# open-mmlab/Amphion

Hardware: AMD Instinct MI355X
Metric: audio samples/sec (HiFi-GAN V1 22.05 kHz generator, mel->wav) (higher is better)
Workload: dtype f32 (split-f16 MFMA: 3 x v_mfma_f32_32x32x16_f16 per term, f32 accumulate)

## Files before the change

amphion_amd/csrc/conv_host.hip:

```cpp
#include <string.h>

#include <memory>
#include <type_traits>
#include <vector>

#include "amp_host.h"

namespace amp {

template <int... K> struct Taps { static constexpr int list[] = {K...}; };
using ConvTaps = Taps<1, 2, 3, 5, 7, 11>;
using BlkTaps = Taps<2, 3, 7, 11>;
using SmallTaps = Taps<1, 3, 5, 7, 11>;
using PairTaps = Taps<3, 5, 7, 11>;
using RbTaps = Taps<3, 5, 7, 11>;
using AmpbTaps = Taps<3, 5, 7, 11>;

template <int... K, typename R, typename F>
static R with_taps(Taps<K...>, int k, R dflt, F&& f) {
    R r = dflt;
    (void)((k == K && (r = f(std::integral_constant<int, K>{}), true)) || ...);
    return r;
}

static hipError_t launch_conv(const ConvPlan& p, const ConvArgs& a, hipStream_t s) {
    return with_taps(ConvTaps{}, p.KT, hipErrorInvalidValue, [&](auto K) { return launch_conv<K>(p, a, s); });
}
static hipError_t launch_conv_f16x3(const ConvPlan& p, const ConvArgs& a, hipStream_t s) {
    return with_taps(ConvTaps{}, p.KT, hipErrorInvalidValue, [&](auto K) { return launch_conv_f16x3<K>(p, a, s); });
}
static int conv_blk_nt(int k, int cm, int halo) { return with_taps(BlkTaps{}, k, 0, [&](auto K) { return conv_blk_nt<K>(cm, halo); }); }
static hipError_t launch_conv_blk(int k, int cm, int wn, const ConvArgs& a, hipStream_t s) {
    return with_taps(BlkTaps{}, k, hipErrorInvalidValue, [&](auto K) { return launch_conv_blk<K>(cm, wn, a, s); });
}
static hipError_t launch_conv_small(int k, int ni, int epi, const ConvArgs& a, hipStream_t s) {
    return with_taps(SmallTaps{}, k, hipErrorInvalidValue, [&](auto K) { return launch_conv_small<K>(ni, epi, a, s); });
}
static int pair_tile(int k, int C, int dil) { return with_taps(PairTaps{}, k, 0, [&](auto K) { return pair_tile<K>(C, dil); }); }
static hipError_t launch_pair(int k, const PairArgs& a, hipStream_t s) {
    return with_taps(PairTaps{}, k, hipErrorInvalidValue, [&](auto K) { return launch_pair<K>(a, s); });
}
static int strip_step(int k, int C, int dil, int wide, int* wg) {
    return with_taps(PairTaps{}, k, 0, [&](auto K) { return strip_step<K>(C, dil, wide, wg); });
}
static hipError_t launch_strip(int k, const PairArgs& a, hipStream_t s) {
    return with_taps(PairTaps{}, k, hipErrorInvalidValue, [&](auto K) { return launch_strip<K>(a, s); });
}
static int rb_tile(int k, int C, int max_dil, int wide) { return with_taps(RbTaps{}, k, 0, [&](auto K) { return rb_tile<K>(C, max_dil, wide); }); }
static hipError_t launch_rb(int k, const RbArgs& a, int wide, hipStream_t s) {
    return with_taps(RbTaps{}, k, hipErrorInvalidValue, [&](auto K) { return launch_rb<K>(a, wide, s); });
}
static int ampb_tile(int k, int C, int max_dil, int wide) {
    return with_taps(AmpbTaps{}, k, 0, [&](auto K) { return ampb_tile<K>(C, max_dil, wide); });
}
static hipError_t launch_ampb(int k, const AmpbArgs& a, int wide, hipStream_t s) {
    return with_taps(AmpbTaps{}, k, hipErrorInvalidValue, [&](auto K) { return launch_ampb<K>(a, wide, s); });
}

static int round_up_taps(int ntaps) {
    for (int kt : ConvTaps::list)
        if (kt >= ntaps) return kt;
    return -1;
}

bool choose_plan(int KT, int M, int halo_total, int , ConvPlan* plan) {
    bool ok = false;
    for (int kt : ConvTaps::list) ok |= (kt == KT);
    if (!ok || halo_total > 128) return false;
    plan->KT = KT;
    plan->HALO = halo_total <= 64 ? 64 : 128;
    if (M > 64) { plan->WM = 4; plan->WN = 1; plan->NI = 8; }
    else if (M > 32) { plan->WM = 2; plan->WN = 2; plan->NI = 8; }
    else { plan->WM = 1; plan->WN = 4; plan->NI = 4; }
    return true;
}

struct StripChoice { bool use; int wide; int steps; };
static StripChoice strip_choice(int C, int k) {
    const int mode = cfg().pair_strips;
    if (mode == 0) return {false, 0, 0};
    if (C == 128 && (k == 7 || k == 11)) return {true, 3, 1};
    return {false, 0, 0};
}

static void strip_plan(int B, int T, int n1, int hb, int wg_per_cu, int* strip_len, int* spi_out) {
    const int slots = wg_per_cu * 256;
    long best = -1; int best_spi = 1;
    const int max_spi = (T + n1 - 1) / n1;
    for (int spi = 1; spi <= max_spi; ++spi) {
        const int L = (T + spi - 1) / spi;
        if ((long)(spi - 1) * L >= T) continue;
        const long steps = (L + hb + n1 - 1) / n1;
        const long rounds = ((long)B * spi + slots - 1) / slots;
        const long cost = rounds * (4 * steps + 1);
        if (best < 0 || cost < best) { best = cost; best_spi = spi; }
    }
    *spi_out = best_spi;
    *strip_len = (T + best_spi - 1) / best_spi;
}

constexpr double kFitPrologueSteps = 0.2;
static void strip_geometry(int B, int T, int n1, int hb, int wg_per_cu, int steps, bool ragged, int* strip_len, int* spi, int* fit) {
    *fit = 0;
    strip_plan(B, T, n1, hb, wg_per_cu, strip_len, spi);
    if (steps > 0 && steps * n1 - hb < T) { *strip_len = steps * n1 - hb; *spi = (T + *strip_len - 1) / *strip_len; }
    bool four = false;
    if (steps == 1 && !ragged && 4 * n1 - hb < T) {
        const int len4 = 4 * n1 - hb, spi4 = (T + len4 - 1) / len4;
        if ((long long)B * spi4 >= 1024) { *strip_len = len4; *spi = spi4; four = true; }
    }
    const int mode = cfg().strip_fit;
    if (mode == 0) return;
    if (mode == 1) {
        const int st = (*strip_len + hb + n1 - 1) / n1;
        *strip_len = st * n1; *spi = (T + *strip_len - 1) / *strip_len; *fit = 1;
        return;
    }
    if (!four) return;
    const long long slots = (long long)wg_per_cu * 256;
    auto rounds = [&](int nspi) { return ((long long)B * nspi + slots - 1) / slots; };
    auto cost = [&](int nspi, double steps_per_strip) { return (double)rounds(nspi) * (4.0 * steps_per_strip + 1.0); };
    double best = cost(*spi, 4.0);
    const long long shifted_rounds = rounds(*spi) * 4;
    for (int S : {4, 8}) {
        const int len = S * n1, nspi = (T + len - 1) / len;
        if (len > T || (long long)B * nspi < 512) continue;
        if (rounds(nspi) * S >= shifted_rounds) continue;
        const double c = cost(nspi, S + kFitPrologueSteps);
        if (c < best) { best = c; *strip_len = len; *spi = nspi; *fit = 1; }
    }
}

bool pair_strip_plan(int B, int T, int k, bool ragged, int* form, int* strip_len, int* spi, int* steps) {
    int wg = 2;
    const StripChoice sc = strip_choice(128, k);
    const int n1 = sc.use ? strip_step(k, 128, 1, sc.wide, &wg) : 0;
    if (n1 <= 0) return false;
    strip_geometry(B, T, n1, k - 1, wg, sc.steps, ragged, strip_len, spi, form);
    *steps = (*strip_len + (*form ? 0 : k - 1) + n1 - 1) / n1;
    return true;
}

constexpr long long kSmallGridWorkgroups = 384;

static bool small_conv_enabled() { return cfg().small_conv != 0; }

static int conv_blk_mode() { return cfg().conv_blk; }
static int narrow_blk_mode() { return cfg().narrow_blk; }
constexpr size_t kConvRgFastMaxWeightBytes = 3u << 20;
static bool conv_rg_fast() { return cfg().conv_rg_fast != 0; }
static thread_local unsigned g_launch_parity = 0;
int next_rev(const int* lens) {
    if (!cfg().pingpong || lens) return 0;
    return (int)(g_launch_parity++ & 1u);
}
constexpr long long kConvBlkMinWorkgroups = 512;

int conv_build(amp_conv* c, const float* w, const float* bias) {
    if (c->cin <= 0 || c->cout <= 0 || c->k <= 0 || c->stride <= 0 || c->dilation <= 0) {
        set_error("amp_conv: bad dimensions cin=%d cout=%d k=%d stride=%d dilation=%d", c->cin, c->cout, c->k, c->stride,
                  c->dilation);
        return AMP_ERR_INVALID;
    }
    if (!c->transposed) {
        if (c->stride != 1) { set_error("amp_conv: strided Conv1d is not on the vocoder path"); return AMP_ERR_UNSUPPORTED; }
        c->up = 1; c->up_pad = 0;
        c->M = c->cout;
        c->ntaps = c->k;
        c->off0 = -c->padding;
        c->dstep = c->dilation;
    } else if (c->stride == 1) {
        if (c->dilation != 1) { set_error("amp_conv: dilated ConvTranspose1d unsupported (dilation=%d)", c->dilation); return AMP_ERR_UNSUPPORTED; }
        c->up = 1; c->up_pad = 0;
        c->M = c->cout;
        c->ntaps = c->k;
        c->off0 = -(c->k - 1 - c->padding);
        c->dstep = 1;
    } else {
        if (c->dilation != 1) { set_error("amp_conv: dilated ConvTranspose1d unsupported (dilation=%d)", c->dilation); return AMP_ERR_UNSUPPORTED; }
        c->up = c->stride; c->up_pad = c->padding;
        c->M = c->cout * c->stride;
        c->ntaps = (c->k + c->stride - 1) / c->stride;
        c->off0 = 0;
        c->dstep = -1;
    }
    c->KT = round_up_taps(c->ntaps);
    if (c->KT < 0) { set_error("amp_conv: k=%d at stride=%d is %d taps, unsupported (max 11)", c->k, c->stride, c->ntaps); return AMP_ERR_UNSUPPORTED; }
    const int omin = c->dstep >= 0 ? c->off0 : c->off0 + (c->KT - 1) * c->dstep;
    const int omax = c->dstep >= 0 ? c->off0 + (c->KT - 1) * c->dstep : c->off0;
    c->halo_left = omin < 0 ? -omin : 0;
    c->halo_right = omax > 0 ? omax : 0;
    if (!choose_plan(c->KT, c->M, c->halo_left + c->halo_right, 0, &c->plan)) {
        set_error("amp_conv: receptive field (k=%d, dilation=%d, padding=%d: %d columns) exceeds the 128-column staged halo", c->k, c->dilation,
                  c->padding, c->halo_left + c->halo_right);
        return AMP_ERR_UNSUPPORTED;
    }
    c->precision = default_precision();
    if (c->precision == PREC_F16X3) c->plan.NI = 4;
    const int Mg = c->plan.Mgroup();
    const int Mpad = ((c->M + Mg - 1) / Mg) * Mg;
    c->Mpad = Mpad;
    const int nmb = Mpad / 32;
    const int cin = c->cin, cout = c->cout, k = c->k, up = c->up;
    auto wview = [&](int m, int i, int g) -> float {
        if (m >= c->M || i >= cin || g >= c->ntaps) return 0.f;
        if (!c->transposed) return w[((size_t)m * cin + i) * k + g];
        if (up == 1) return w[((size_t)i * cout + m) * k + (k - 1 - g)];
        const int o = m / up, r = m - o * up;
        const int j = r + g * up;
        return j < k ? w[((size_t)i * cout + o) * k + j] : 0.f;
    };
    if (c->precision == PREC_F32) {
        c->nchunks = (c->cin + KC - 1) / KC;
        const size_t n = ((size_t)nmb * c->nchunks + 1) * c->KT * 64 * 4;
        std::vector<float> wp(n, 0.f);
        for (int mb = 0; mb < nmb; ++mb)
            for (int ch = 0; ch < c->nchunks; ++ch)
                for (int g = 0; g < c->KT; ++g)
                    for (int lane = 0; lane < 64; ++lane)
                        for (int p = 0; p < 4; ++p)
                            wp[((((size_t)mb * c->nchunks + ch) * c->KT + g) * 64 + lane) * 4 + p] =
                                wview(mb * 32 + (lane & 31), ch * KC + 2 * p + (lane >> 5), g);
        AMP_RC(device_upload(wp.data(), n * sizeof(float), &c->wp_dev));
    } else {
        c->nchunks = (c->cin + KC16 - 1) / KC16;
        float wmax = 0.f;
        const size_t nw = (size_t)cin * cout * k;
        for (size_t i = 0; i < nw; ++i) wmax = fmaxf(wmax, fabsf(w[i]));
        if (!(wmax < 1e30f)) { set_error("amp_conv: non-finite weight"); return AMP_ERR_INVALID; }
        c->wscale = pow2_weight_scale(wmax);
        const std::vector<_Float16> wp = pack_a_f16x3(nmb, c->nchunks, c->KT, (size_t)2 * c->KT * 2, c->wscale, wview);
        AMP_RC(device_upload(wp.data(), wp.size() * sizeof(_Float16), &c->wp_dev));
    }
    if (bias) AMP_RC(device_upload(bias, (size_t)cout * sizeof(float), (void**)&c->bias_dev));
    return AMP_OK;
}

static size_t conv_weight_bytes(const amp_conv* c) { return (size_t)c->Mpad * c->nchunks * KC16 * c->KT * 4; }

static int conv_out_len(const amp_conv* c, int T) {
    if (!c->transposed) return T + 2 * c->padding - c->dilation * (c->k - 1);
    return (T - 1) * c->stride - 2 * c->padding + c->k + c->out_pad;
}

static bool small_conv_static_ok(const amp_conv* c) {
    return c->precision == PREC_F16X3 && !c->transposed && !c->pad_reflect && c->plan.WM == 4 &&
           (c->KT == 1 || c->KT == 3 || c->KT == 5 || c->KT == 7 || c->KT == 11) && c->KT == c->ntaps &&
           c->nchunks <= kSmallConvMaxChunks && c->halo_left + c->halo_right <= 64;
}
static bool small_conv_covers(const amp_conv* c) { return small_conv_enabled() && small_conv_static_ok(c); }
static int small_conv_ni(const amp_conv* c) { return (c->halo_left + c->halo_right <= 32) ? 1 : 2; }

int conv_run(const amp_conv* c, const float* x, int B, int T, float slope_in, const float* res, float slope_out,
             float* y, int mode, float div, hipStream_t stream, long long xbs, const int* lens, int len_mul,
             ConvArgs* plan_small, int* plan_ni) {
    if (B <= 0 || T <= 0) { set_error("amp_conv_forward: B=%d T=%d", B, T); return AMP_ERR_INVALID; }
    const int Tout = conv_out_len(c, T);
    if (Tout <= 0) { set_error("amp_conv_forward: input too short (T=%d gives T_out=%d)", T, Tout); return AMP_ERR_INVALID; }
    ConvArgs a{};
    a.x = x; a.wp = c->wp_dev; a.bias = c->bias_dev; a.res = res; a.y = y;
    a.B = B; a.Cin = c->cin; a.Tin = T; a.xbs = xbs > 0 ? xbs : (long long)c->cin * T; a.nchunks = c->nchunks; a.M = c->M;
    a.Tq = c->up > 1 ? T + c->ntaps - 1 : Tout;
    ConvPlan plan = c->plan;
    if (c->precision == PREC_F16X3) {
        const long long wgs = (long long)B * ((a.Tq + plan.NT() - 1) / plan.NT()) * ((c->M + plan.Mgroup() - 1) / plan.Mgroup());
        if (wgs < kSmallGridWorkgroups) plan.NI = 2;
    }
    const int NT = plan.NT();
    a.tiles_per_item = (a.Tq + NT - 1) / NT;
    a.off0 = c->off0; a.dstep = c->dstep; a.halo_left = c->halo_left;
    a.wd = NT + c->halo_left + c->halo_right;
    a.Cout = c->cout; a.Tout = Tout; a.up = c->up; a.up_pad = c->up_pad;
    a.slope_in = slope_in; a.slope_out = slope_out; a.mode = mode; a.div = div;
    a.lens = lens; a.len_mul = len_mul;
    a.pad_reflect = c->pad_reflect; a.tanh_out = c->tanh_out;
    a.range_flag = c->precision == PREC_F16X3 ? range_flag_for_current_device() : nullptr;
    a.rev = c->precision == PREC_F16X3 ? next_rev(lens) : 0;
    if (c->pad_reflect && (c->halo_left >= T || c->halo_right >= T)) {
        set_error("amp_conv_forward: reflection padding %d needs more than %d input samples", c->halo_left > c->halo_right ? c->halo_left : c->halo_right, T);
        return AMP_ERR_INVALID;
    }
    if (c->gated_H) { set_error("amp_conv_forward: a gated conv (amp_conv_create_gated) only runs inside amp_wn_forward"); return AMP_ERR_STATE; }
    if (c->precision == PREC_F16X3 && slope_in > 1.f) {
        set_error("amp_conv_forward: leaky_relu slope %g > 1 on the input is outside the f16x3 kernels (use AMP_PRECISION_F32)", (double)slope_in);
        return AMP_ERR_UNSUPPORTED;
    }
    tl_conv_transposed = c->transposed;
    if (c->precision == PREC_F32) {
        if (plan_small) return AMP_ERR_UNSUPPORTED;
        a.acc_scale = a.inv_scale = 1.f;
        AMP_HIP(launch_conv(plan, a, stream));
    } else {
        a.acc_scale = 16.f * c->wscale;
        a.inv_scale = 1.f / a.acc_scale;
        const long long wgs_half = (long long)B * ((a.Tq + 63) / 64) * ((c->M + plan.Mgroup() - 1) / plan.Mgroup());
        int blk_cm = 0, blk_nt = 0, blk_wn = 1;
        const bool blk_kt = c->KT == 2 || c->KT == 3 || (conv_blk_mode() == 3 && (c->KT == 7 || c->KT == 11));
        if (c->M % 256 == 0) blk_wn = 1;
        else if (c->M % 128 == 0 && c->KT != 2 && (narrow_blk_mode() >= 2 || (narrow_blk_mode() == 1 && c->KT >= 7))) blk_wn = 2;
        else blk_wn = 0;
        if (conv_blk_mode() > 0 && plan.NI == 4 && blk_wn > 0 && blk_kt && !c->tanh_out && !c->pad_reflect) {
            int cm = (conv_blk_mode() >= 2 && c->KT == 2 && c->nchunks % 2 == 0) ? 2 : 1;
            const int halo = c->halo_left + c->halo_right;
            const int nt = blk_wn * conv_blk_nt(c->KT, cm, halo);
            if (nt > 0 && (long long)B * ((a.Tq + nt - 1) / nt) * (c->M / (256 / blk_wn)) >= kConvBlkMinWorkgroups) { blk_cm = cm; blk_nt = nt; }
        }
        if (plan_small && !(blk_cm == 0 && plan.NI == 2 && small_conv_covers(c) && (c->KT <= 5 || wgs_half <= 128))) return AMP_ERR_UNSUPPORTED;
        if (blk_cm > 0) {
            const int rows = 256 / blk_wn;
            a.tiles_per_item = (a.Tq + blk_nt - 1) / blk_nt;
            a.wd = blk_nt + c->halo_left + c->halo_right;
            a.row_groups = (conv_rg_fast() && c->M / rows > 1 && conv_weight_bytes(c) <= kConvRgFastMaxWeightBytes) ? c->M / rows : 0;
            AMP_HIP(launch_conv_blk(c->KT, blk_cm, blk_wn, a, stream));
        } else if (plan.NI == 2 && small_conv_covers(c) && (c->KT <= 5 || wgs_half <= 128)) {
            const int ni = small_conv_ni(c);
            a.Mpad = c->Mpad;
            a.tiles_per_item = (a.Tq + 32 * ni - 1) / (32 * ni);
            a.wd = 32 * ni + c->halo_left + c->halo_right;
            if (plan_small) { *plan_small = a; *plan_ni = ni; return AMP_OK; }
            AMP_HIP(launch_conv_small(c->KT, ni, 0, a, stream));
        } else {
            const int nrg = (c->M + plan.Mgroup() - 1) / plan.Mgroup();
            a.row_groups = (conv_rg_fast() && nrg > 1 && conv_weight_bytes(c) <= kConvRgFastMaxWeightBytes) ? nrg : 0;
            AMP_HIP(launch_conv_f16x3(plan, a, stream));
        }
    }
    return AMP_OK;
}

bool pair_supported(const amp_conv* c1, const amp_conv* c2) {
    if (c1->precision != PREC_F16X3 || c2->precision != PREC_F16X3) return false;
    if (c1->pad_reflect || c2->pad_reflect || c1->tanh_out || c2->tanh_out) return false;
    if (c1->transposed || c2->transposed || c1->cin != c1->cout || c2->cin != c2->cout || c1->cin != c2->cin) return false;
    if (c1->k != c2->k || c2->dilation != 1 || c1->k != c1->KT) return false;
    if (c1->padding != (c1->k - 1) / 2 * c1->dilation || c2->padding != (c2->k - 1) / 2) return false;
    if (!c1->bias_dev || !c2->bias_dev) return false;
    const StripChoice sc = strip_choice(c1->cin, c1->k);
    if (sc.use && strip_step(c1->k, c1->cin, c1->dilation, sc.wide, nullptr) > 0) return true;
    return pair_tile(c1->k, c1->cin, c1->dilation) > 0;
}

int pair_run(const amp_conv* c1, const amp_conv* c2, const float* x, int B, int T, float slope, float* y,
                    int mode, float div, hipStream_t stream, const int* lens, int len_mul) {
    if (x == y) { set_error("pair_run: x and y must not alias"); return AMP_ERR_INVALID; }
    if (slope > 1.f) { set_error("pair_run: leaky_relu slope %g > 1 is outside the fused pair kernels", (double)slope); return AMP_ERR_UNSUPPORTED; }
    PairArgs a{};
    a.x = x; a.y = y;
    a.wp1 = c1->wp_dev; a.bias1 = c1->bias_dev; a.wp2 = c2->wp_dev; a.bias2 = c2->bias_dev;
    a.B = B; a.C = c1->cin; a.T = T;
    a.dil = c1->dilation;
    a.slope = slope;
    a.sc1 = 16.f * c1->wscale; a.isc1 = 1.f / a.sc1;
    a.sc2 = 16.f * c2->wscale; a.isc2 = 1.f / a.sc2;
    a.mode = mode; a.div = div;
    a.lens = lens; a.len_mul = len_mul;
    a.range_flag = range_flag_for_current_device();
    a.rev = next_rev(lens);
    int wg = 2;
    const StripChoice sc = strip_choice(c1->cin, c1->k);
    const int n1 = sc.use ? strip_step(c1->k, c1->cin, c1->dilation, sc.wide, &wg) : 0;
    if (n1 > 0) {
        a.wide = sc.wide;
        strip_geometry(B, T, n1, c1->k - 1, wg, sc.steps, lens != nullptr, &a.strip_len, &a.strips_per_item, &a.fit);
        if (cfg().pair_strips == -1 && sc.wide >= 2 && (long long)B * a.strips_per_item < 512 && pair_tile(c1->k, c1->cin, c1->dilation) > 0) {
            const int NT = pair_tile(c1->k, c1->cin, c1->dilation);
            a.tiles_per_item = (T + NT - 1) / NT;
            AMP_HIP(launch_pair(c1->k, a, stream));
            return AMP_OK;
        }
        AMP_HIP(launch_strip(c1->k, a, stream));
        return AMP_OK;
    }
    const int NT = pair_tile(c1->k, c1->cin, c1->dilation);
    a.tiles_per_item = (T + NT - 1) / NT;
    AMP_HIP(launch_pair(c1->k, a, stream));
    return AMP_OK;
}

bool pair_tile_args(const amp_conv* c1, const amp_conv* c2, const float* x, int B, int T, float slope, float* y, int mode,
                           float div, const int* lens, int len_mul, PairArgs* out) {
    if (x == y || slope > 1.f || !pair_supported(c1, c2)) return false;
    PairArgs a{};
    a.x = x; a.y = y;
    a.wp1 = c1->wp_dev; a.bias1 = c1->bias_dev; a.wp2 = c2->wp_dev; a.bias2 = c2->bias_dev;
    a.B = B; a.C = c1->cin; a.T = T;
    a.dil = c1->dilation;
    a.slope = slope;
    a.sc1 = 16.f * c1->wscale; a.isc1 = 1.f / a.sc1;
    a.sc2 = 16.f * c2->wscale; a.isc2 = 1.f / a.sc2;
    a.mode = mode; a.div = div;
    a.lens = lens; a.len_mul = len_mul;
    a.range_flag = range_flag_for_current_device();
    a.rev = 0;
    int wg = 2;
    const StripChoice sc = strip_choice(c1->cin, c1->k);
    const int n1 = sc.use ? strip_step(c1->k, c1->cin, c1->dilation, sc.wide, &wg) : 0;
    if (n1 > 0) {
        int strip_len = 0, strips_per_item = 0, fit = 0;
        strip_geometry(B, T, n1, c1->k - 1, wg, sc.steps, lens != nullptr, &strip_len, &strips_per_item, &fit);
        if (!(cfg().pair_strips == -1 && sc.wide >= 2 && (long long)B * strips_per_item < 512)) return false;
    }
    const int NT = pair_tile(c1->k, c1->cin, c1->dilation);
    if (NT <= 0) return false;
    a.tiles_per_item = (T + NT - 1) / NT;
    *out = a;
    return true;
}

static int rb_fusion_mode() { return cfg().rb_fusion; }
static int rb_form(int C, int k) {
    const int m = rb_fusion_mode();
    if (m == 0) return -1;
    if (m == 3) return (C == 32 || (C == 64 && k <= 5)) ? 0 : 1;
    if (m == 2) return 1;
    if (C == 32) return k >= 11 ? 1 : 0;
    if (C == 64) return k <= 5 ? 0 : 1;
    if (C == 128) return 1;
    return -1;
}
constexpr long long kRbMinWorkgroups = 256;

bool rb_supported(const amp_conv* const* c1, const amp_conv* const* c2, int np, int B, int T) {
    if (np < 1 || np > AMP_RB_MAX_PAIRS) return false;
    int max_dil = 1, rh = 0;
    for (int p = 0; p < np; ++p) {
        if (!c1[p] || !c2[p] || !pair_supported(c1[p], c2[p])) return false;
        if (c1[p]->cin != c1[0]->cin || c1[p]->k != c1[0]->k) return false;
        max_dil = c1[p]->dilation > max_dil ? c1[p]->dilation : max_dil;
        rh += (c1[p]->k - 1) / 2 * (c1[p]->dilation + 1);
    }
    const int form = rb_form(c1[0]->cin, c1[0]->k);
    if (form < 0) return false;
    const int W = rb_tile(c1[0]->k, c1[0]->cin, max_dil, form);
    if (W <= 0 || W - 2 * rh < W / 2) return false;
    const int NT = W - 2 * rh;
    if (rb_fusion_mode() == 1 && (long long)B * ((T + NT - 1) / NT) < kRbMinWorkgroups) return false;
    return true;
}

int rb_split(const amp_conv* const* c1, int np, int B, int T) {
    if (np != 3 || rb_fusion_mode() != 1) return 0;
    int max_dil = 1, rh = 0;
    for (int p = 0; p < np; ++p) {
        max_dil = c1[p]->dilation > max_dil ? c1[p]->dilation : max_dil;
        rh += (c1[p]->k - 1) / 2 * (c1[p]->dilation + 1);
    }
    const int W = rb_tile(c1[0]->k, c1[0]->cin, max_dil, rb_form(c1[0]->cin, c1[0]->k));
    const int NT = W - 2 * rh;
    if (W <= 0 || 5 * NT >= 4 * W) return 0;
    if ((long long)B * ((T + NT - 1) / NT) < 1024) return 0;
    return 2;
}

int rb_run(const amp_conv* const* c1, const amp_conv* const* c2, int np, const float* x, int B, int T, float slope, float* y, int mode,
           float div, hipStream_t stream, const int* lens, int len_mul, int first, int count) {
    if (x == y) { set_error("rb_run: x and y must not alias"); return AMP_ERR_INVALID; }
    if (slope > 1.f) { set_error("rb_run: leaky_relu slope %g > 1 is outside the fused kernels", (double)slope); return AMP_ERR_UNSUPPORTED; }
    RbArgs a{};
    a.x = x; a.y = y;
    a.np = count < 0 ? np - first : count;
    c1 += first;
    c2 += first;
    int max_dil = 1;
    for (int p = 0; p < a.np; ++p) {
        a.wp1[p] = c1[p]->wp_dev; a.bias1[p] = c1[p]->bias_dev; a.wp2[p] = c2[p]->wp_dev; a.bias2[p] = c2[p]->bias_dev;
        a.sc1[p] = 16.f * c1[p]->wscale; a.isc1[p] = 1.f / a.sc1[p];
        a.sc2[p] = 16.f * c2[p]->wscale; a.isc2[p] = 1.f / a.sc2[p];
        a.dil[p] = c1[p]->dilation;
        a.rh += (c1[p]->k - 1) / 2 * (c1[p]->dilation + 1);
        max_dil = c1[p]->dilation > max_dil ? c1[p]->dilation : max_dil;
    }
    for (int p = a.np; p < AMP_RB_MAX_PAIRS; ++p) {
        a.wp1[p] = a.wp1[0]; a.bias1[p] = a.bias1[0]; a.wp2[p] = a.wp2[0]; a.bias2[p] = a.bias2[0]; a.dil[p] = 1;
    }
    a.B = B; a.C = c1[0]->cin; a.T = T;
    const int form = rb_form(a.C, c1[0]->k);
    const int W = rb_tile(c1[0]->k, a.C, max_dil, form);
    const int NT = W - 2 * a.rh;
    a.tiles_per_item = (T + NT - 1) / NT;
    a.slope = slope; a.mode = mode; a.div = div;
    a.lens = lens; a.len_mul = len_mul;
    a.range_flag = range_flag_for_current_device();
    a.rev = next_rev(lens);
    AMP_HIP(launch_rb(c1[0]->k, a, form, stream));
    return AMP_OK;
}

static int ampb_fusion_mode() { return cfg().ampb_fusion; }
static int ampb_form(int C, int k) {
    const int m = ampb_fusion_mode();
    if (m == 0) return -1;
    if (m == 3) return C == 32 ? 0 : 1;
    if (m == 2) return 1;
    if (C == 32) return k >= 11 ? 1 : 0;
    if (C == 64) return k <= 3 ? 1 : -1;
    return -1;
}
constexpr long long kAmpbMinWorkgroups = 256;

static int ampb_halo(const amp_conv* const* c1, int np) {
    int rh = 0;
    for (int p = 0; p < np; ++p) rh += 10 + (c1[p]->k - 1) / 2 * (c1[p]->dilation + 1);
    return (rh + 3) & ~3;
}

bool ampb_supported(const amp_conv* const* c1, const amp_conv* const* c2, int np, const ActParams* acts, size_t nacts, int B, int T) {
    if (np < 1 || 2 * np > AMP_AMPB_MAX_STEPS || nacts != (size_t)(2 * np)) return false;
    for (size_t i = 0; i < nacts; ++i)
        if (!acts[i].fu2_dev) return false;
    if ((T & 3) != 0) return false;
    int max_dil = 1;
    for (int p = 0; p < np; ++p) {
        const amp_conv *a = c1[p], *b = c2[p];
        if (!a || !b || a->precision != PREC_F16X3 || b->precision != PREC_F16X3) return false;
        if (a->pad_reflect || b->pad_reflect || a->tanh_out || b->tanh_out || a->transposed || b->transposed) return false;
        if (a->cin != a->cout || b->cin != b->cout || a->cin != b->cin || a->cin != c1[0]->cin) return false;
        if (a->k != c1[0]->k || b->k != a->k || b->dilation != 1 || a->k != a->KT) return false;
        if (a->padding != (a->k - 1) / 2 * a->dilation || b->padding != (b->k - 1) / 2) return false;
        if (!a->bias_dev || !b->bias_dev) return false;
        max_dil = a->dilation > max_dil ? a->dilation : max_dil;
    }
    const int form = ampb_form(c1[0]->cin, c1[0]->k);
    if (form < 0) return false;
    const int W = ampb_tile(c1[0]->k, c1[0]->cin, max_dil, form);
    const int rh = ampb_halo(c1, np);
    if (W <= 0 || W - 2 * rh < W / 2) return false;
    const int NT = W - 2 * rh;
    if (ampb_fusion_mode() == 1 && (long long)B * ((T + NT - 1) / NT) < kAmpbMinWorkgroups) return false;
    return true;
}

int ampb_run(const amp_conv* const* c1, const amp_conv* const* c2, int np, const ActParams* acts, const float* x, int B, int T,
                    float* y, int mode, float div, hipStream_t stream, const int* lens, int len_mul) {
    if (x == y) { set_error("ampb_run: x and y must not alias"); return AMP_ERR_INVALID; }
    AmpbArgs a{};
    a.x = x; a.y = y;
    a.ns = 2 * np;
    int max_dil = 1;
    for (int s = 0; s < AMP_AMPB_MAX_STEPS; ++s) {
        const int sv = s < a.ns ? s : 0;
        const amp_conv* c = (sv & 1) ? c2[sv >> 1] : c1[sv >> 1];
        a.wp[s] = c->wp_dev; a.bias[s] = c->bias_dev;
        a.sc[s] = 16.f * c->wscale; a.isc[s] = 1.f / a.sc[s];
        a.dil[s] = c->dilation;
        a.act_a[s] = acts[sv].a_dev; a.act_invb[s] = acts[sv].invb_dev; a.act_fu[s] = acts[sv].fu2_dev; a.act_fd[s] = acts[sv].fd_dev;
        max_dil = c->dilation > max_dil ? c->dilation : max_dil;
    }
    a.rh = ampb_halo(c1, np);
    a.B = B; a.C = c1[0]->cin; a.T = T;
    const int form = ampb_form(a.C, c1[0]->k);
    const int W = ampb_tile(c1[0]->k, a.C, max_dil, form);
    const int NT = W - 2 * a.rh;
    a.tiles_per_item = (T + NT - 1) / NT;
    a.mode = mode; a.div = div;
    a.lens = lens; a.len_mul = len_mul;
    a.range_flag = range_flag_for_current_device();
    a.rev = next_rev(lens);
    AMP_HIP(launch_ampb(c1[0]->k, a, form, stream));
    return AMP_OK;
}

int act_params_upload(const float* alpha_dev, const float* beta_dev, int C, int logscale, const float* filt_up_host,
                             const float* filt_down_host, float** out) {
    std::vector<float> al(C), be(C), a(C), ib(C);
    AMP_HIP(hipMemcpy(al.data(), alpha_dev, C * sizeof(float), hipMemcpyDeviceToHost));
    if (beta_dev) AMP_HIP(hipMemcpy(be.data(), beta_dev, C * sizeof(float), hipMemcpyDeviceToHost));
    for (int i = 0; i < C; ++i) {
        float av = al[i], bv = beta_dev ? be[i] : al[i];
        if (logscale) { av = expf(av); bv = expf(bv); }
        a[i] = av;
        ib[i] = 1.0f / (bv + 0.000000001f);
    }
    float* scratch = nullptr;
    AMP_HIP(hipMalloc((void**)&scratch, (2 * (size_t)C + 36) * sizeof(float)));
    float fu2[12];
    for (int i = 0; i < 12; ++i) fu2[i] = 2.f * filt_up_host[i];
    hipError_t e = hipMemcpy(scratch, a.data(), C * sizeof(float), hipMemcpyHostToDevice);
    if (e == hipSuccess) e = hipMemcpy(scratch + C, ib.data(), C * sizeof(float), hipMemcpyHostToDevice);
    if (e == hipSuccess) e = hipMemcpy(scratch + 2 * C, filt_up_host, 12 * sizeof(float), hipMemcpyHostToDevice);
    if (e == hipSuccess) e = hipMemcpy(scratch + 2 * C + 12, filt_down_host, 12 * sizeof(float), hipMemcpyHostToDevice);
    if (e == hipSuccess) e = hipMemcpy(scratch + 2 * C + 24, fu2, 12 * sizeof(float), hipMemcpyHostToDevice);
    if (e != hipSuccess) { (void)hipFree(scratch); set_error("act_params_upload: %s", hipGetErrorString(e)); return AMP_ERR_HIP; }
    *out = scratch;
    return AMP_OK;
}

}

using namespace amp;

extern "C" {

int amp_conv_create(int transposed, int cin, int cout, int k, int stride, int dilation, int padding,
                    const float* weight_host, const float* bias_host, amp_conv** out) {
    if (!weight_host || !out) { set_error("amp_conv_create: null argument"); return AMP_ERR_INVALID; }
    if (amp_device_count() <= 0) { set_error("amp_conv_create: no HIP device visible (the HIP path has no CPU fallback)"); return AMP_ERR_HIP; }
    auto c = std::make_unique<amp_conv>();
    c->transposed = transposed; c->cin = cin; c->cout = cout; c->k = k; c->stride = stride; c->dilation = dilation; c->padding = padding;
    int rc = conv_build(c.get(), weight_host, bias_host);
    if (rc != AMP_OK) return rc;
    *out = c.release();
    return AMP_OK;
}

int amp_conv_create_gated(int hidden, int k, int dilation, int padding, const float* weight_host, const float* bias_host,
                          amp_conv** out) {
    if (!weight_host || !out) { set_error("amp_conv_create_gated: null argument"); return AMP_ERR_INVALID; }
    if (amp_device_count() <= 0) { set_error("amp_conv_create_gated: no HIP device visible (the HIP path has no CPU fallback)"); return AMP_ERR_HIP; }
    if (hidden <= 0 || hidden % 32 != 0) { set_error("amp_conv_create_gated: hidden=%d must be a multiple of 32", hidden); return AMP_ERR_UNSUPPORTED; }
    if (default_precision() != PREC_F16X3) { set_error("amp_conv_create_gated: the fused WN layer exists for the f16x3 arithmetic only"); return AMP_ERR_UNSUPPORTED; }
    const int H = hidden, M = 2 * H;
    const size_t rowlen = (size_t)H * k;
    std::vector<float> wperm((size_t)M * rowlen), bperm((size_t)M, 0.f);
    for (int p = 0; p < M; ++p) {
        const int mb = p >> 5, rho = p & 31;
        const int i = rho & 3, hi = (rho >> 2) & 1, jj = rho >> 3, s = jj & 1, u = jj >> 1;
        const int orow = s * H + 16 * mb + i + 4 * hi + 8 * u;
        memcpy(&wperm[(size_t)p * rowlen], &weight_host[(size_t)orow * rowlen], rowlen * sizeof(float));
        if (bias_host) bperm[p] = bias_host[orow];
    }
    auto c = std::make_unique<amp_conv>();
    c->transposed = 0; c->cin = H; c->cout = M; c->k = k; c->stride = 1; c->dilation = dilation; c->padding = padding;
    int rc = conv_build(c.get(), wperm.data(), bperm.data());
    if (rc != AMP_OK) return rc;
    if (!small_conv_static_ok(c.get()) || conv_out_len(c.get(), 64) != 64) {
        set_error("amp_conv_create_gated: H=%d k=%d dilation=%d padding=%d is outside the fused WN kernel (k in {1,3,5}, H <= 256, 'same' padding, (k-1)*dilation <= 64)", H, k, dilation, padding);
        return AMP_ERR_UNSUPPORTED;
    }
    c->gated_H = H;
    *out = c.release();
    return AMP_OK;
}

static void small_args(const amp_conv* c, const float* x, int B, int T, const int* lens, int ni, ConvArgs* a) {
    *a = ConvArgs{};
    a->x = x; a->wp = c->wp_dev; a->bias = c->bias_dev;
    a->B = B; a->Cin = c->cin; a->Tin = T; a->xbs = (long long)c->cin * T; a->nchunks = c->nchunks; a->M = c->M; a->Mpad = c->Mpad;
    a->Tq = T; a->tiles_per_item = (T + 32 * ni - 1) / (32 * ni);
    a->off0 = c->off0; a->dstep = c->dstep; a->halo_left = c->halo_left; a->wd = 32 * ni + c->halo_left + c->halo_right;
    a->Cout = c->cout; a->Tout = T; a->up = 1; a->up_pad = 0;
    a->slope_in = 1.f; a->slope_out = 1.f; a->mode = 0; a->div = 1.f;
    a->lens = lens; a->len_mul = 1;
    a->acc_scale = 16.f * c->wscale; a->inv_scale = 1.f / a->acc_scale;
    a->range_flag = range_flag_for_current_device();
}

int amp_wn_forward(const amp_conv* const* in_layers, const amp_conv* const* res_skip_layers, int n_layers, float* x_dev,
                   const float* cond_dev, long long cond_batch_stride, const int32_t* lens_dev, int B, int T,
                   float* acts_ws_dev, float* out_dev, void* stream_) {
    if (!in_layers || !res_skip_layers || n_layers <= 0 || !x_dev || !acts_ws_dev || !out_dev || B <= 0 || T <= 0) {
        set_error("amp_wn_forward: bad argument");
        return AMP_ERR_INVALID;
    }
    hipStream_t stream = (hipStream_t)stream_;
    const int H = in_layers[0] ? in_layers[0]->gated_H : 0;
    for (int i = 0; i < n_layers; ++i) {
        const amp_conv* ci = in_layers[i];
        const amp_conv* cr = res_skip_layers[i];
        if (!ci || !cr) { set_error("amp_wn_forward: null layer %d", i); return AMP_ERR_INVALID; }
        const int rs_out = i < n_layers - 1 ? 2 * H : H;
        if (!ci->gated_H || ci->gated_H != H || cr->k != 1 || cr->cin != H || cr->cout != rs_out || cr->gated_H ||
            !small_conv_static_ok(cr) || cr->tanh_out || ci->tanh_out || !cr->bias_dev || !ci->bias_dev) {
            set_error("amp_wn_forward: layer %d is not an (amp_conv_create_gated in-layer, 1x1 %d -> %d res_skip) pair", i, H, rs_out);
            return AMP_ERR_INVALID;
        }
    }
    for (int i = 0; i < n_layers; ++i) {
        ConvArgs a;
        const int ni_in = small_conv_ni(in_layers[i]), ni_rs = small_conv_ni(res_skip_layers[i]);
        small_args(in_layers[i], x_dev, B, T, lens_dev, ni_in, &a);
        a.y = acts_ws_dev; a.wn_H = H;
        a.gate_cond = cond_dev ? cond_dev + (size_t)i * 2 * H : nullptr;
        a.gate_cond_bs = cond_batch_stride;
        AMP_HIP(launch_conv_small(in_layers[i]->KT, ni_in, 1, a, stream));
        small_args(res_skip_layers[i], acts_ws_dev, B, T, nullptr, ni_rs, &a);
        a.lens = lens_dev;
        a.wn_H = H; a.wn_x = x_dev; a.wn_out = out_dev; a.wn_first = i == 0; a.wn_last = i == n_layers - 1;
        AMP_HIP(launch_conv_small(1, ni_rs, 2, a, stream));
    }
    return AMP_OK;
}

int amp_conv_out_len(const amp_conv* c, int T) { return c ? conv_out_len(c, T) : 0; }

int amp_conv_forward(const amp_conv* c, const float* x_dev, int B, int T, float slope_in, const float* res_dev,
                     float slope_out, float* y_dev, void* stream) {
    if (!c || !x_dev || !y_dev) { set_error("amp_conv_forward: null argument"); return AMP_ERR_INVALID; }
    if (x_dev == y_dev) { set_error("amp_conv_forward: x and y must not alias (the conv reads a halo)"); return AMP_ERR_INVALID; }
    return conv_run(c, x_dev, B, T, slope_in, res_dev, slope_out, y_dev, 0, 1.f, (hipStream_t)stream);
}

int amp_conv_forward_strided(const amp_conv* c, const float* x_dev, long long x_batch_stride, int B, int T,
                             float slope_in, const float* res_dev, float slope_out, float* y_dev, void* stream) {
    if (!c || !x_dev || !y_dev) { set_error("amp_conv_forward_strided: null argument"); return AMP_ERR_INVALID; }
    if (x_batch_stride < (long long)c->cin * T) { set_error("amp_conv_forward_strided: batch stride %lld < cin*T", x_batch_stride); return AMP_ERR_INVALID; }
    return conv_run(c, x_dev, B, T, slope_in, res_dev, slope_out, y_dev, 0, 1.f, (hipStream_t)stream, x_batch_stride);
}

int amp_conv_forward_ragged(const amp_conv* c, const float* x_dev, long long x_batch_stride, int B, int T, const int32_t* lens_dev,
                            float slope_in, const float* res_dev, float slope_out, float* y_dev, void* stream) {
    if (!c || !x_dev || !y_dev) { set_error("amp_conv_forward_ragged: null argument"); return AMP_ERR_INVALID; }
    if (x_dev == y_dev) { set_error("amp_conv_forward_ragged: x and y must not alias (the conv reads a halo)"); return AMP_ERR_INVALID; }
    if (x_batch_stride != 0 && x_batch_stride < (long long)c->cin * T) { set_error("amp_conv_forward_ragged: batch stride %lld < cin*T", x_batch_stride); return AMP_ERR_INVALID; }
    if (lens_dev && (c->transposed || c->pad_reflect || conv_out_len(c, T) != T)) {
        set_error("amp_conv_forward_ragged: valid lengths need a 'same' zero-padded Conv1d (output length == input length)");
        return AMP_ERR_UNSUPPORTED;
    }
    return conv_run(c, x_dev, B, T, slope_in, res_dev, slope_out, y_dev, 0, 1.f, (hipStream_t)stream, x_batch_stride, lens_dev);
}

int amp_pair_forward(const amp_conv* c1, const amp_conv* c2, const float* x_dev, int B, int T, float slope,
                     float* y_dev, void* stream) {
    if (!c1 || !c2 || !x_dev || !y_dev) { set_error("amp_pair_forward: null argument"); return AMP_ERR_INVALID; }
    if (B <= 0 || T <= 0) { set_error("amp_pair_forward: B=%d T=%d", B, T); return AMP_ERR_INVALID; }
    if (!pair_supported(c1, c2)) {
        set_error("amp_pair_forward: pair (C=%d k=%d dilation=%d) is not covered by the fused kernel", c1->cin, c1->k, c1->dilation);
        return AMP_ERR_UNSUPPORTED;
    }
    return pair_run(c1, c2, x_dev, B, T, slope, y_dev, 0, 1.f, (hipStream_t)stream);
}

int amp_resblock_forward(const amp_conv* const* c1, const amp_conv* const* c2, int n_pairs, const float* x_dev, int B, int T,
                         float slope, float* y_dev, void* stream) {
    if (!c1 || !c2 || !x_dev || !y_dev) { set_error("amp_resblock_forward: null argument"); return AMP_ERR_INVALID; }
    if (B <= 0 || T <= 0 || n_pairs < 1 || n_pairs > AMP_RB_MAX_PAIRS) { set_error("amp_resblock_forward: B=%d T=%d n_pairs=%d", B, T, n_pairs); return AMP_ERR_INVALID; }
    for (int p = 0; p < n_pairs; ++p) if (!c1[p] || !c2[p]) { set_error("amp_resblock_forward: null conv handle"); return AMP_ERR_INVALID; }
    if (!rb_supported(c1, c2, n_pairs, B, T)) {
        set_error("amp_resblock_forward: block (C=%d k=%d, %d pairs, B=%d T=%d) is not covered by the whole-resblock kernel under the "
                  "current amp_set_resblock_fusion mode", c1[0]->cin, c1[0]->k, n_pairs, B, T);
        return AMP_ERR_UNSUPPORTED;
    }
    return rb_run(c1, c2, n_pairs, x_dev, B, T, slope, y_dev, 0, 1.f, (hipStream_t)stream);
}

int amp_ampblock_forward(const amp_conv* const* c1, const amp_conv* const* c2, int n_pairs, const float* alpha_dev,
                         const float* beta_dev, int logscale, const float* filt_up_host, const float* filt_down_host,
                         const float* x_dev, int B, int T, float* y_dev, int mode, float div, void* stream) {
    if (!c1 || !c2 || !alpha_dev || !filt_up_host || !filt_down_host || !x_dev || !y_dev) { set_error("amp_ampblock_forward: null argument"); return AMP_ERR_INVALID; }
    if (B <= 0 || T <= 0 || n_pairs < 1 || 2 * n_pairs > AMP_AMPB_MAX_STEPS || mode < 0 || mode > 2) {
        set_error("amp_ampblock_forward: B=%d T=%d n_pairs=%d mode=%d", B, T, n_pairs, mode);
        return AMP_ERR_INVALID;
    }
    if (x_dev == y_dev) { set_error("amp_ampblock_forward: x and y must not alias (tiles read each other's halo)"); return AMP_ERR_INVALID; }
    for (int p = 0; p < n_pairs; ++p) if (!c1[p] || !c2[p]) { set_error("amp_ampblock_forward: null conv handle"); return AMP_ERR_INVALID; }
    const int C = c1[0]->cin, na = 2 * n_pairs;
    float* scratch[AMP_AMPB_MAX_STEPS] = {};
    ActParams acts[AMP_AMPB_MAX_STEPS];
    int rc = AMP_OK;
    for (int i = 0; i < na && rc == AMP_OK; ++i) {
        rc = act_params_upload(alpha_dev + (size_t)i * C, beta_dev ? beta_dev + (size_t)i * C : nullptr, C, logscale, filt_up_host, filt_down_host, &scratch[i]);
        if (rc == AMP_OK) { acts[i].a_dev = scratch[i]; acts[i].invb_dev = scratch[i] + C; acts[i].fu_dev = scratch[i] + 2 * C; acts[i].fd_dev = scratch[i] + 2 * C + 12; acts[i].fu2_dev = scratch[i] + 2 * C + 24; }
    }
    if (rc == AMP_OK && !ampb_supported(c1, c2, n_pairs, acts, (size_t)na, B, T)) {
        set_error("amp_ampblock_forward: block (C=%d k=%d, %d pairs, B=%d T=%d) is not covered by the whole-AMPBlock kernel under the "
                  "current amp_set_ampblock_fusion mode (run the convs and activations one by one: the same bits)", c1[0]->cin, c1[0]->k, n_pairs, B, T);
        rc = AMP_ERR_UNSUPPORTED;
    }
    if (rc == AMP_OK) rc = ampb_run(c1, c2, n_pairs, acts, x_dev, B, T, y_dev, mode, div, (hipStream_t)stream);
    hipError_t e = hipStreamSynchronize((hipStream_t)stream);
    for (int i = 0; i < na; ++i) if (scratch[i]) (void)hipFree(scratch[i]);
    if (rc == AMP_OK && e != hipSuccess) { set_error("amp_ampblock_forward: %s", hipGetErrorString(e)); return AMP_ERR_HIP; }
    return rc;
}

int amp_conv_forward_mrf(const amp_conv* c, const float* x_dev, int B, int T, float slope_in, const float* res_dev,
                         float* y_dev, int mode, float div, void* stream) {
    if (!c || !x_dev || !y_dev) { set_error("amp_conv_forward_mrf: null argument"); return AMP_ERR_INVALID; }
    if (x_dev == y_dev) { set_error("amp_conv_forward_mrf: x and y must not alias (the conv reads a halo)"); return AMP_ERR_INVALID; }
    if (mode < 0 || mode > 2 || (mode == 2 && !(div > 0.f))) { set_error("amp_conv_forward_mrf: mode=%d div=%g", mode, (double)div); return AMP_ERR_INVALID; }
    return conv_run(c, x_dev, B, T, slope_in, res_dev, 1.f, y_dev, mode, div, (hipStream_t)stream);
}

int amp_conv_set_option(amp_conv* c, int option, int value) {
    if (!c) { set_error("amp_conv_set_option: null handle"); return AMP_ERR_INVALID; }
    if (option == AMP_CONV_OPT_PAD_REFLECT) {
        if (value && c->transposed) { set_error("amp_conv_set_option: reflection padding on a transposed conv"); return AMP_ERR_UNSUPPORTED; }
        c->pad_reflect = value != 0;
    } else if (option == AMP_CONV_OPT_TANH) {
        if (value && c->transposed) { set_error("amp_conv_set_option: tanh on a transposed conv"); return AMP_ERR_UNSUPPORTED; }
        c->tanh_out = value != 0;
    } else {
        set_error("amp_conv_set_option: unknown option %d", option);
        return AMP_ERR_INVALID;
    }
    return AMP_OK;
}

void amp_conv_destroy(amp_conv* c) { delete c; }

}
```

amphion_amd/csrc/rb_f16x3.hip:

```cpp
#include "f16x3_device.h"

#ifndef AMP_KT
#error "compile with -DAMP_KT=<taps>"
#endif

namespace amp {


template <int KT, int WM, int WN, int NI, int RING = 0, int RB_G = 32>
__global__ __launch_bounds__(64 * WM * WN, 2) void rb_f16x3_kernel(const RbArgs a) {
    static_assert(RING == 0 || RING < KT, "a ring shorter than one chunk");
    constexpr int NTHR = 64 * WM * WN;
    constexpr int W = 32 * NI * WN;
    constexpr int WL = W + 2 * RB_G;
    constexpr int H2 = (KT - 1) / 2;
    constexpr int NCH = 2 * WM;
    constexpr int CHS = 4 * WL;
    constexpr int C = 32 * WM;
    static_assert(NI % 2 == 0, "B fragments are read in halves");
    extern __shared__ __attribute__((aligned(16))) uint4 smem4[];

    const int tid = threadIdx.x;
    const int lane = tid & 63;
    const int wave = __builtin_amdgcn_readfirstlane(tid >> 6);
    const int wm = wave / WN, wn = wave % WN;
    const int hi = lane >> 5, l31 = lane & 31;
    const int nbx = gridDim.x;
    int bx = tile_order(blockIdx.x, nbx, a.lens != nullptr, a.rev);
    const int item = bx / a.tiles_per_item;
    const int tile = bx - item * a.tiles_per_item;
    const int T = a.T;
    const int RH = a.rh;
    const int NT = W - 2 * RH;
    const int O0 = tile * NT;
    int Tv = T;
    if (a.lens) { const int l = a.lens[item] * a.len_mul; Tv = l < Tv ? l : Tv; }
    if (O0 >= Tv) return;
    const int q0 = O0 - RH;

    for (int i = tid; i < NCH * 4 * 2 * RB_G; i += NTHR) {
        const int row = i / (2 * RB_G), g = i - row * (2 * RB_G);
        smem4[row * WL + (g < RB_G ? g : W + g)] = make_uint4(0u, 0u, 0u, 0u);
    }

    const int colw = wn * (32 * NI) + l31;
    int qcl[NI];
    bool qok[NI];
#pragma unroll
    for (int t = 0; t < NI; ++t) {
        const int q = q0 + colw + 32 * t;
        qok[t] = (q >= 0) && (q < Tv);
        qcl[t] = q < 0 ? 0 : (q < T ? q : T - 1);
    }
    const float* xr = a.x + (size_t)item * C * T + (size_t)(32 * wm + 16 * hi) * T;
    f32x16 rv[NI];
#pragma unroll
    for (int t = 0; t < NI; ++t)
#pragma unroll
        for (int r = 0; r < 16; ++r) rv[t][r] = xr[(size_t)r * T + qcl[t]];

    constexpr size_t MBS = (size_t)NCH * (KT * 128);
    constexpr int NA = RING > 0 ? RING : KT;
    Frag a_h[NA], a_l[NA];
    const int wlane = (lane & 32) | (16 * ((lane >> 2) & 1) + 4 * ((lane >> 3) & 3) + (lane & 3));
    {
        const uint4* w0 = static_cast<const uint4*>(a.wp1[0]) + (size_t)wm * MBS + wlane;
#pragma unroll
        for (int g = 0; g < NA; ++g) {
            a_h[g].u = w0[g * 128];
            a_l[g].u = w0[g * 128 + 64];
        }
    }
    AMP_PIN_VMEM();

    float range_max = 0.f;
    const float kpos = 16.f, kneg = 16.f * a.slope;
    auto stage_x = [&]() __attribute__((always_inline)) {
#pragma unroll
        for (int t = 0; t < NI; ++t) {
            const int col = RB_G + colw + 32 * t;
            const bool ok = qok[t];
            const int o4 = (2 * wm + hi) * CHS + col;
#pragma unroll
            for (int o = 0; o < 2; ++o) {
                struct { uint2 u; } fh0, fl0, fh1, fl1;
                stage4_f16(ok ? rv[t][8 * o + 0] : 0.f, ok ? rv[t][8 * o + 1] : 0.f, ok ? rv[t][8 * o + 2] : 0.f,
                           ok ? rv[t][8 * o + 3] : 0.f, kpos, kneg, range_max, fh0.u, fl0.u);
                stage4_f16(ok ? rv[t][8 * o + 4] : 0.f, ok ? rv[t][8 * o + 5] : 0.f, ok ? rv[t][8 * o + 6] : 0.f,
                           ok ? rv[t][8 * o + 7] : 0.f, kpos, kneg, range_max, fh1.u, fl1.u);
                smem4[o4 + o * WL] = make_uint4(fh0.u.x, fh0.u.y, fh1.u.x, fh1.u.y);
                smem4[o4 + o * WL + 2 * WL] = make_uint4(fl0.u.x, fl0.u.y, fl1.u.x, fl1.u.y);
            }
        }
    };

    f32x16 acc[NI];
    auto conv = [&](const void* wp, const float* bias, float sc, int d, const void* wp_next) __attribute__((always_inline)) {
#pragma unroll
        for (int r = 0; r < 16; ++r) {
            const float bv = bias[32 * wm + 16 * hi + r] * sc;
#pragma unroll
            for (int t = 0; t < NI; ++t) acc[t][r] = bv;
        }
        const uint4* wa = static_cast<const uint4*>(wp) + (size_t)wm * MBS + wlane;
        const uint4* wn0 = static_cast<const uint4*>(wp_next) + (size_t)wm * MBS + wlane;
        const int rd = hi * WL + RB_G + colw - H2 * d;
#pragma unroll 1
        for (int c = 0; c < NCH; ++c) {
            const uint4* wcur = wa + (size_t)c * (KT * 128);
            const uint4* wan = (c + 1) < NCH ? wa + (size_t)(c + 1) * (KT * 128) : wn0;
            const uint4* base = smem4 + c * CHS + rd;
#pragma unroll
            for (int g = 0; g < KT; ++g) {
                const int v = RING > 0 ? g % NA : g;
                const uint4* bg = base + g * d;
                constexpr int NB = NI / 2;
#pragma unroll
                for (int th = 0; th < 2; ++th) {
                    Frag bh[NB], bl[NB];
#pragma unroll
                    for (int t = 0; t < NB; ++t) {
                        bh[t].u = bg[32 * (th * NB + t)];
                        bl[t].u = bg[2 * WL + 32 * (th * NB + t)];
                    }
                    mfma3<NB>(acc + th * NB, a_h[v], a_l[v], bh, bl);
                }
                {
                    const bool same = RING > 0 && g + RING < KT;
                    const uint4* src = same ? wcur + (size_t)(g + RING) * 128 : wan + (size_t)v * 128;
                    a_h[v].u = src[0];
                    a_l[v].u = src[64];
                }
                AMP_PIN_VMEM();
            }
        }
    };

    stage_x();
    __syncthreads();

    const int np = a.np;
#pragma unroll 1
    for (int p = 0; p < AMP_RB_MAX_PAIRS; ++p) {
        if (p < np) {
            const bool last = (p + 1 == np);
            conv(a.wp1[p], a.bias1[p], a.sc1[p], a.dil[p], a.wp2[p]);
            __syncthreads();
            {
                const float i1 = a.isc1[p];
                const float slope = a.slope;
#pragma unroll
                for (int t = 0; t < NI; ++t) {
                    const int o4 = (2 * wm + hi) * CHS + RB_G + colw + 32 * t;
#pragma unroll
                    for (int o = 0; o < 2; ++o) {
                        struct { uint2 u; } fh0, fl0, fh1, fl1;
                        seam4_f16(acc[t][8 * o + 0], acc[t][8 * o + 1], acc[t][8 * o + 2], acc[t][8 * o + 3], i1, slope, qok[t], range_max, fh0.u, fl0.u);
                        seam4_f16(acc[t][8 * o + 4], acc[t][8 * o + 5], acc[t][8 * o + 6], acc[t][8 * o + 7], i1, slope, qok[t], range_max, fh1.u, fl1.u);
                        smem4[o4 + o * WL] = make_uint4(fh0.u.x, fh0.u.y, fh1.u.x, fh1.u.y);
                        smem4[o4 + o * WL + 2 * WL] = make_uint4(fl0.u.x, fl0.u.y, fl1.u.x, fl1.u.y);
                    }
                }
            }
            __syncthreads();
            conv(a.wp2[p], a.bias2[p], a.sc2[p], 1, last ? a.wp2[p] : a.wp1[p + 1 < AMP_RB_MAX_PAIRS ? p + 1 : p]);
            {
                const float i2 = a.isc2[p];
#pragma unroll
                for (int t = 0; t < NI; ++t)
#pragma unroll
                    for (int r = 0; r < 16; ++r) rv[t][r] = __builtin_fmaf(acc[t][r], i2, rv[t][r]);
            }
            if (!last) {
                __syncthreads();
                stage_x();
                __syncthreads();
            }
        }
    }

    {
        const int mode = a.mode;
        float* yr = a.y + (size_t)item * C * T + (size_t)(32 * wm + 16 * hi) * T;
        if (mode != 0) {
#pragma unroll
            for (int t = 0; t < NI; ++t)
#pragma unroll
                for (int r = 0; r < 16; ++r) acc[t][r] = yr[(size_t)r * T + qcl[t]];
#pragma unroll
            for (int t = 0; t < NI; ++t) rv[t] += acc[t];
            if (mode == 2) {
#pragma unroll
                for (int t = 0; t < NI; ++t)
#pragma unroll
                    for (int r = 0; r < 16; ++r) rv[t][r] = rv[t][r] / a.div;
            }
        }
#pragma unroll
        for (int t = 0; t < NI; ++t) {
            const int col = colw + 32 * t;
            const int q = q0 + col;
            if (col >= RH && col < W - RH && q < T) {
#pragma unroll
                for (int r = 0; r < 16; ++r) yr[(size_t)r * T + qcl[t]] = rv[t][r];
            }
        }
    }
    if (a.range_flag && __any(range_max > 65504.f) && lane == 0) atomicOr(a.range_flag, 1u);
}

template <int KT, int WM, int WN, int NI, int RING = 0, int RB_G = 32>
static hipError_t launch_rb_one(const RbArgs& a, hipStream_t stream) {
    constexpr int W = 32 * NI * WN;
    const size_t lds = (size_t)2 * WM * 4 * (W + 2 * RB_G) * sizeof(uint4);
    if (hipError_t e = ensure_dynamic_lds<&rb_f16x3_kernel<KT, WM, WN, NI, RING, RB_G>>(lds); e != hipSuccess) return e;
    dim3 grid((unsigned)(a.B * a.tiles_per_item));
    note_kernel("rb_f16x3_kernel", KT, WM, WN, NI, RING, RB_G);
    note_work(grid.x, a.np * 2 * 2.0 * a.C * a.C * KT * (double)a.T * a.B / 1e9, 4.0 * a.B * (double)a.C * a.T * (2 + (a.mode ? 1 : 0)) / 1e6,
              "whole ResBlock C=%d k=%d T=%d B=%d: %d convs%s", a.C, KT, a.T, a.B, 2 * a.np, a.mode ? " +sum" : "");
    hipLaunchKernelGGL((rb_f16x3_kernel<KT, WM, WN, NI, RING, RB_G>), grid, dim3(64 * WM * WN), lds, stream, a);
    return hipGetLastError();
}

template <int KT>
int rb_tile(int C, int max_dil, int wide) {
    const int reach = (KT - 1) / 2 * max_dil;
    if (reach > 32) return 0;
    if (C == 32) return wide ? 1024 : 512;
    if (C == 64) return wide ? 512 : ((KT <= 5 && reach <= 16) ? 256 : 0);
    if (C == 128) return (wide && KT <= 5 && reach <= 16) ? 256 : 0;
    return 0;
}

template <int KT>
hipError_t launch_rb(const RbArgs& a, int wide, hipStream_t stream) {
    constexpr int RING = KT >= 7 ? 4 : 0;
    if (a.C == 32) return wide ? launch_rb_one<KT, 1, 8, 4, RING>(a, stream) : launch_rb_one<KT, 1, 4, 4, RING>(a, stream);
    if (a.C == 64 && wide) return launch_rb_one<KT, 2, 4, 4, RING>(a, stream);
    if constexpr (KT <= 5) {
        if (a.C == 64 && !wide) return launch_rb_one<KT, 2, 2, 4, 0, 16>(a, stream);
    }
    if constexpr (KT <= 5) {
        if (a.C == 128 && wide) return launch_rb_one<KT, 4, 2, 4, 0, 16>(a, stream);
    }

    return hipErrorInvalidValue;
}

template int rb_tile<AMP_KT>(int, int, int);
template hipError_t launch_rb<AMP_KT>(const RbArgs&, int, hipStream_t);

}
```

Before: 153.6 million.

## Load first-conv halo into ResBlock guard columns to shrink tile overlap

```diff
diff --git a/amphion_amd/csrc/conv_host.hip b/amphion_amd/csrc/conv_host.hip
--- a/amphion_amd/csrc/conv_host.hip
+++ b/amphion_amd/csrc/conv_host.hip
@@ -420,34 +420,57 @@
 }
 constexpr long long kRbMinWorkgroups = 256;
 
+struct RbPlan {
+    int form;
+    int W;
+    int G;
+    int rf;
+    int rh;
+    int NT;
+    int tiles_per_item;
+};
+static RbPlan rb_plan(const amp_conv* const* c1, int np, int T) {
+    RbPlan pl{};
+    const int C = c1[0]->cin, k = c1[0]->k;
+    int max_dil = 1;
+    for (int p = 0; p < np; ++p) {
+        max_dil = c1[p]->dilation > max_dil ? c1[p]->dilation : max_dil;
+        pl.rf += (k - 1) / 2 * (c1[p]->dilation + 1);
+    }
+    pl.form = rb_form(C, k);
+    if (pl.form < 0) return pl;
+    pl.W = rb_tile(k, C, max_dil, pl.form);
+    if (pl.W <= 0 && pl.form == 0) {
+        pl.form = 1;
+        pl.W = rb_tile(k, C, max_dil, 1);
+    }
+    if (pl.W <= 0) { pl.W = 0; return pl; }
+    pl.G = (C == 128 || (C == 64 && pl.form == 0)) ? 16 : 32;
+    pl.rh = pl.rf - (k - 1) / 2 * c1[0]->dilation;
+    pl.NT = pl.W - 2 * pl.rh;
+    if (pl.NT <= 0 || (k - 1) / 2 * c1[0]->dilation > pl.G) { pl.W = 0; return pl; }
+    pl.tiles_per_item = (T + pl.NT - 1) / pl.NT;
+    return pl;
+}
+
 bool rb_supported(const amp_conv* const* c1, const amp_conv* const* c2, int np, int B, int T) {
     if (np < 1 || np > AMP_RB_MAX_PAIRS) return false;
-    int max_dil = 1, rh = 0;
     for (int p = 0; p < np; ++p) {
         if (!c1[p] || !c2[p] || !pair_supported(c1[p], c2[p])) return false;
         if (c1[p]->cin != c1[0]->cin || c1[p]->k != c1[0]->k) return false;
-        max_dil = c1[p]->dilation > max_dil ? c1[p]->dilation : max_dil;
-        rh += (c1[p]->k - 1) / 2 * (c1[p]->dilation + 1);
-    }
-    const int form = rb_form(c1[0]->cin, c1[0]->k);
-    if (form < 0) return false;
-    const int W = rb_tile(c1[0]->k, c1[0]->cin, max_dil, form);
-    if (W <= 0 || W - 2 * rh < W / 2) return false;
-    const int NT = W - 2 * rh;
-    if (rb_fusion_mode() == 1 && (long long)B * ((T + NT - 1) / NT) < kRbMinWorkgroups) return false;
+    }
+    const RbPlan pl = rb_plan(c1, np, T);
+    if (pl.W <= 0 || pl.NT < pl.W / 2) return false;
+    if (rb_fusion_mode() == 1 && (long long)B * pl.tiles_per_item < kRbMinWorkgroups) return false;
     return true;
 }
 
 int rb_split(const amp_conv* const* c1, int np, int B, int T) {
     if (np != 3 || rb_fusion_mode() != 1) return 0;
-    int max_dil = 1, rh = 0;
-    for (int p = 0; p < np; ++p) {
-        max_dil = c1[p]->dilation > max_dil ? c1[p]->dilation : max_dil;
-        rh += (c1[p]->k - 1) / 2 * (c1[p]->dilation + 1);
-    }
-    const int W = rb_tile(c1[0]->k, c1[0]->cin, max_dil, rb_form(c1[0]->cin, c1[0]->k));
-    const int NT = W - 2 * rh;
-    if (W <= 0 || 5 * NT >= 4 * W) return 0;
+    const RbPlan pl = rb_plan(c1, np, T);
+    if (pl.W <= 0) return 0;
+    const int NT = pl.W - 2 * pl.rf;
+    if (NT <= 0 || 5 * NT >= 4 * pl.W) return 0;
     if ((long long)B * ((T + NT - 1) / NT) < 1024) return 0;
     return 2;
 }
@@ -461,28 +484,25 @@
     a.np = count < 0 ? np - first : count;
     c1 += first;
     c2 += first;
-    int max_dil = 1;
     for (int p = 0; p < a.np; ++p) {
         a.wp1[p] = c1[p]->wp_dev; a.bias1[p] = c1[p]->bias_dev; a.wp2[p] = c2[p]->wp_dev; a.bias2[p] = c2[p]->bias_dev;
         a.sc1[p] = 16.f * c1[p]->wscale; a.isc1[p] = 1.f / a.sc1[p];
         a.sc2[p] = 16.f * c2[p]->wscale; a.isc2[p] = 1.f / a.sc2[p];
         a.dil[p] = c1[p]->dilation;
-        a.rh += (c1[p]->k - 1) / 2 * (c1[p]->dilation + 1);
-        max_dil = c1[p]->dilation > max_dil ? c1[p]->dilation : max_dil;
     }
     for (int p = a.np; p < AMP_RB_MAX_PAIRS; ++p) {
         a.wp1[p] = a.wp1[0]; a.bias1[p] = a.bias1[0]; a.wp2[p] = a.wp2[0]; a.bias2[p] = a.bias2[0]; a.dil[p] = 1;
     }
     a.B = B; a.C = c1[0]->cin; a.T = T;
-    const int form = rb_form(a.C, c1[0]->k);
-    const int W = rb_tile(c1[0]->k, a.C, max_dil, form);
-    const int NT = W - 2 * a.rh;
-    a.tiles_per_item = (T + NT - 1) / NT;
+    const RbPlan pl = rb_plan(c1, a.np, T);
+    if (pl.W <= 0) { set_error("rb_run: no whole-ResBlock tile for C = %d, k = %d and these dilations", a.C, c1[0]->k); return AMP_ERR_UNSUPPORTED; }
+    a.rh = pl.rh;
+    a.tiles_per_item = pl.tiles_per_item;
     a.slope = slope; a.mode = mode; a.div = div;
     a.lens = lens; a.len_mul = len_mul;
     a.range_flag = range_flag_for_current_device();
     a.rev = next_rev(lens);
-    AMP_HIP(launch_rb(c1[0]->k, a, form, stream));
+    AMP_HIP(launch_rb(c1[0]->k, a, pl.form, stream));
     return AMP_OK;
 }
 
diff --git a/amphion_amd/csrc/rb_f16x3.hip b/amphion_amd/csrc/rb_f16x3.hip
--- a/amphion_amd/csrc/rb_f16x3.hip
+++ b/amphion_amd/csrc/rb_f16x3.hip
@@ -38,9 +38,35 @@
     if (O0 >= Tv) return;
     const int q0 = O0 - RH;
 
-    for (int i = tid; i < NCH * 4 * 2 * RB_G; i += NTHR) {
-        const int row = i / (2 * RB_G), g = i - row * (2 * RB_G);
-        smem4[row * WL + (g < RB_G ? g : W + g)] = make_uint4(0u, 0u, 0u, 0u);
+    float range_max = 0.f;
+    const float kpos = 16.f, kneg = 16.f * a.slope;
+
+    {
+        const int gf = H2 * a.dil[0];
+        const float* xi = a.x + (size_t)item * C * T;
+        for (int i = tid; i < NCH * 2 * 2 * RB_G; i += NTHR) {
+            const int row = i / (2 * RB_G), g = i - row * (2 * RB_G);
+            const int col = g < RB_G ? g : W + g;
+            uint4 vh = make_uint4(0u, 0u, 0u, 0u), vl = vh;
+            if (g < RB_G ? g >= RB_G - gf : g < RB_G + gf) {
+                const int q = q0 + col - RB_G;
+                const bool ok = (q >= 0) && (q < Tv);
+                const float* xg = xi + (size_t)(8 * row) * T + (q < 0 ? 0 : (q < T ? q : T - 1));
+                float v[8];
+#pragma unroll
+                for (int r = 0; r < 8; ++r) v[r] = xg[(size_t)r * T];
+#pragma unroll
+                for (int r = 0; r < 8; ++r) v[r] = ok ? v[r] : 0.f;
+                struct { uint2 u; } fh0, fl0, fh1, fl1;
+                stage4_f16(v[0], v[1], v[2], v[3], kpos, kneg, range_max, fh0.u, fl0.u);
+                stage4_f16(v[4], v[5], v[6], v[7], kpos, kneg, range_max, fh1.u, fl1.u);
+                vh = make_uint4(fh0.u.x, fh0.u.y, fh1.u.x, fh1.u.y);
+                vl = make_uint4(fl0.u.x, fl0.u.y, fl1.u.x, fl1.u.y);
+            }
+            const int o4 = (row >> 1) * CHS + (row & 1) * WL + col;
+            smem4[o4] = vh;
+            smem4[o4 + 2 * WL] = vl;
+        }
     }
 
     const int colw = wn * (32 * NI) + l31;
@@ -73,8 +99,6 @@
     }
     AMP_PIN_VMEM();
 
-    float range_max = 0.f;
-    const float kpos = 16.f, kneg = 16.f * a.slope;
     auto stage_x = [&]() __attribute__((always_inline)) {
 #pragma unroll
         for (int t = 0; t < NI; ++t) {
```

Result: no change. 154.8 million (median of 6 runs) (+0.8%).
